# microsoft/typeagent-py

Measured on AMD Instinct MI355X. Metric: queries/sec + p50 lookup latency, 1536-d top-32 kNN at 1/2/4/8 MI355X, higher is better.
Workload: dtype f16 storage, f32 accumulate; 1 GPU; cfg3: 10000000x1536 fp16, 1024 q/step, top-32, min_score 0; total_rows=10000000, k=32, parallelism=single GPU

## Files before the change

include/tavb.h:

```cpp
#ifndef TAVB_H
#define TAVB_H

#include <stdint.h>

#ifdef __cplusplus
extern "C" {
#endif

#define TAVB_ABI_VERSION 7

#define TAVB_OK 0
#define TAVB_E_INVALID (-1)
#define TAVB_E_HIP (-2)
#define TAVB_E_NO_CORPUS (-3)
#define TAVB_E_UNSUPPORTED (-4)
#define TAVB_E_NOMEM (-5)
#define TAVB_E_TIMEOUT (-7)
#define TAVB_E_PEER (-6)

#define TAVB_F32 0
#define TAVB_F16 1

#define TAVB_MAX_FUSED_K 256
#define TAVB_MAX_LARGE_K 16384
// ... 98 lines not shown
#define TAVB_KERNEL_MFMA 2
#define TAVB_KERNEL_NORMALIZE 3
#define TAVB_KERNEL_CONVERT 4
#define TAVB_KERNEL_MFMA_SAMPLE 5
#define TAVB_KERNEL_SKINNY 6
#define TAVB_KERNEL_RESCORE 7
#define TAVB_KERNEL_EXCHANGE 8
#define TAVB_KERNEL_TOPK 9
#define TAVB_KERNEL_COUNT 10
int tavb_profile_enable(tavb_ctx* ctx, int32_t on);
int tavb_profile_reset(tavb_ctx* ctx);
int tavb_profile_read(tavb_ctx* ctx, int32_t kernel_id, double* out_total_ms, int64_t* out_launches);

int tavb_plan_ladder(int64_t rows, int32_t nq, int32_t n_cu, int64_t* out_bounds, int32_t cap);

#ifdef __cplusplus
}
#endif
#endif
```

typeagent_py_amd/_native.py:

```python

from __future__ import annotations

import ctypes
import os
import threading
from ctypes import POINTER, byref, c_char_p, c_double, c_float, c_int, c_int32, c_int64, c_uint64, c_void_p

import numpy as np

ABI_VERSION = 7
TAVB_F32 = 0
TAVB_F16 = 1
MAX_FUSED_K = 256
MAX_LARGE_K = 16384
MAX_STREAM_QUERIES = 8

KERNEL_SCAN, KERNEL_MERGE, KERNEL_MFMA, KERNEL_NORMALIZE, KERNEL_CONVERT, KERNEL_MFMA_SAMPLE, KERNEL_SKINNY, KERNEL_RESCORE, KERNEL_EXCHANGE, KERNEL_TOPK = range(10)
COMM_ID_BYTES = 128

_LIB_NAME = os.environ.get("TAVB_LIBRARY", "libtavb.so")
_lib = None
_lib_lock = threading.Lock()

_SIGNATURES = [
# ... 37 lines not shown
    ("tavb_search_device", c_int, [c_void_p, c_void_p, c_int32, c_int32, c_float, c_void_p]),
    ("tavb_search_subset_device", c_int, [c_void_p, c_void_p, c_void_p, c_int64, c_int32, c_float, c_void_p]),
    ("tavb_search_subset_resident", c_int, [c_void_p, c_void_p, c_void_p, c_int64, c_int32, c_float, c_void_p, c_void_p, c_void_p]),
    ("tavb_merge_device", c_int, [c_void_p, c_void_p, c_int32, c_int32, c_int32, c_void_p]),
    ("tavb_decode_keys", c_int, [c_void_p, c_int32, c_int32, c_void_p, c_void_p, c_void_p]),
    ("tavb_comm_unique_id", c_int, [c_void_p]),
    ("tavb_comm_init", c_int, [c_void_p, c_void_p, c_int32, c_int32]),
    ("tavb_comm_destroy", c_int, [c_void_p]),
    ("tavb_search_allgather", c_int, [c_void_p, c_void_p, c_int32, c_int32, c_float, c_void_p]),
    ("tavb_allgather_merge", c_int, [c_void_p, c_void_p, c_int32, c_int32, c_void_p]),
    ("tavb_remap_key_positions", c_int, [c_void_p, c_void_p, c_int64, c_void_p, c_int64]),
    ("tavb_profile_enable", c_int, [c_void_p, c_int32]),
    ("tavb_profile_reset", c_int, [c_void_p]),
    ("tavb_profile_read", c_int, [c_void_p, c_int32, POINTER(c_double), POINTER(c_int64)]),
    ("tavb_plan_ladder", c_int, [c_int64, c_int32, c_int32, POINTER(c_int64), c_int32]),
]

ABI_SYMBOLS = [name for name, _, _ in _SIGNATURES]


_AS_POINTER = ctypes.c_char * 0


def _addr(arr: np.ndarray):
    try:
        return _AS_POINTER.from_buffer(arr)
    except (TypeError, ValueError, BufferError):
        return arr.ctypes.data_as(c_void_p)


def plan_ladder(rows: int, nq: int, n_cu: int = 256) -> list[int]:
    lib = load_library(preload_torch=False)
    buf = (c_int64 * 16)()
    n = lib.tavb_plan_ladder(int(rows), int(nq), int(n_cu), buf, 16)
    _check(lib, n if n < 0 else 0)
    return [int(buf[i]) for i in range(n + 1)]


def library_path() -> str:
    return os.path.join(os.path.dirname(os.path.abspath(__file__)), _LIB_NAME)


def load_library(preload_torch: bool = True):
    global _lib
    with _lib_lock:
        if _lib is not None:
            return _lib
        path = library_path()
        if not os.path.isfile(path):
            raise RuntimeError(
                f"{path} is missing: build it with `python -c 'import __graft_entry__ as g; g.build()'` "
# ... 558 lines not shown
```

typeagent_py_amd/csrc/tavb_abi.hip:

```cpp

#include <hip/hip_runtime.h>
#include <dlfcn.h>
#include <rccl/rccl.h>

#include <algorithm>
#include <atomic>
#include <chrono>
#include <functional>
#include <mutex>
#include <cmath>
#include <cstdarg>
#include <cstdio>
#include <cstring>
#include <string>
#include <thread>
#include <vector>

#include "tavb_internal.h"

typedef unsigned long long u64_t;

namespace {

thread_local std::string g_last_error;
// ... 118 lines not shown
  Buffer d_sort_keys, d_sort_ws;
  Buffer h_sort_info{nullptr, 0, true};
  int64_t sort_all = 1;
  int64_t sort_stage_keys = (int64_t)1 << 21;
  int64_t sort_small_keys = 16384;
  Buffer h_ring[2] = {{nullptr, 0, true}, {nullptr, 0, true}};
  Buffer d_ring[2];
  hipEvent_t ring_done[2] = {nullptr, nullptr};
  const int32_t* row_to_msg = nullptr;
  int64_t row_to_msg_rows = 0, n_messages = 0;
  int64_t norm_rows = 0;
  Buffer h_stage{nullptr, 0, true};
  Buffer h_out{nullptr, 0, true};
  Buffer h_lists{nullptr, 0, true};
  Buffer h_flag{nullptr, 0, true};
  int64_t mfma_bdirect = 0;
  int64_t band_max = tavb::kBandMax;
  int64_t early_exact = 1;
  int64_t wide_fallback = 1;
  int64_t small_direct_bytes = (int64_t)128 << 20;
  int64_t small_direct_keys = 8192;
  int64_t last_direct = 0;
  int inline_query = 1;
  int64_t direct_group_max_nq = TAVB_MAX_GROUPED_QUERIES;
  int64_t direct_group = 0;
  int64_t direct_group_wgs = 0;
  bool dispatch_no_group = false;
  int64_t direct_group_keys = 32768;

  bool profiling = false;
// ... 435 lines not shown
  } else if (n == "mfma_ablate") {
    if (v < 0 || v > 4095) return fail(TAVB_E_INVALID, "mfma_ablate must be 0..4095");
    c->mfma_ablate = v;
  } else if (n == "mfma_splits") {
    if (v < 0 || v > 4096) return fail(TAVB_E_INVALID, "mfma_splits out of range");
    c->mfma_splits = v;
  } else if (n == "band_max") {
    if (v < TAVB_MAX_FUSED_K || v > tavb::kBandMax) return fail(TAVB_E_INVALID, "band_max must be %d .. %d", TAVB_MAX_FUSED_K, tavb::kBandMax);
    c->band_max = v;
  } else if (n == "early_exact") {
    c->early_exact = v ? 1 : 0;
  } else if (n == "wide_fallback") {
    c->wide_fallback = v ? 1 : 0;
  } else if (n == "mfma_bdirect") {
    c->mfma_bdirect = v ? 1 : 0;
  } else if (n == "small_direct_keys") {
    if (v < 64 || v > (1 << 20)) return fail(TAVB_E_INVALID, "small_direct_keys must be 64 .. 1048576");
    c->small_direct_keys = v;
  } else if (n == "inline_query") {
    c->inline_query = v ? 1 : 0;
  } else if (n == "direct_group_max_nq") {
    if (v < 0 || v > TAVB_MAX_GROUPED_QUERIES) return fail(TAVB_E_INVALID, "direct_group_max_nq must be 0 .. %d", TAVB_MAX_GROUPED_QUERIES);
    c->direct_group_max_nq = v;
  } else if (n == "direct_group") {
    if (!(v == 0 || v == 1 || v == 2 || v == 4 || v == 8)) return fail(TAVB_E_INVALID, "direct_group must be 0, 1, 2, 4 or 8");
    c->direct_group = v;
  } else if (n == "direct_group_wgs") {
    if (v != 0 && (v < 8 || v > 65536)) return fail(TAVB_E_INVALID, "direct_group_wgs must be 0 or 8 .. 65536");
    c->direct_group_wgs = v;
  } else if (n == "direct_group_keys") {
// ... 83 lines not shown
  else if (n == "small_direct_bytes") *out = c->small_direct_bytes;
  else if (n == "wide_fallback") *out = c->wide_fallback;
  else if (n == "early_exact") *out = c->early_exact;
  else if (n == "band_max") *out = c->band_max;
  else if (n == "last_doomed") {
    *out = 0;
    if (c->d_flag.ptr) {
      DeviceGuard guard(c->device);
      int v = 0;
      TAVB_HIP(hipStreamSynchronize(c->stream));
      TAVB_HIP(hipMemcpy(&v, reinterpret_cast<const int*>(c->d_flag.ptr) + 1, sizeof v, hipMemcpyDeviceToHost));
      *out = v;
    }
  }
  else if (n == "mfma_bdirect") *out = c->mfma_bdirect;
  else if (n == "last_direct") *out = c->last_direct;
  else if (n == "inline_query") *out = c->inline_query;
  else if (n == "small_direct_keys") *out = c->small_direct_keys;
  else if (n == "direct_group_max_nq") *out = c->direct_group_max_nq;
  else if (n == "direct_group") *out = c->direct_group;
  else if (n == "direct_group_wgs") *out = c->direct_group_wgs;
  else if (n == "direct_group_keys") *out = c->direct_group_keys;
  else if (n == "graph_max_bytes") *out = c->graph_max_bytes;
  else if (n == "last_graph") *out = c->last_graph;
  else if (n == "large_k") *out = c->large_k;
  else if (n == "topk_buckets") *out = c->topk_buckets;
  else if (n == "topk_boundary_keys") *out = c->topk_boundary_keys;
  else if (n == "topk_scores_bytes") *out = c->topk_scores_bytes;
  else if (n == "last_topk_refine") *out = c->last_topk_refine;
  else if (n == "sort_all") *out = c->sort_all;
// ... 1496 lines not shown
  p.nq_padded = r.nq_pad;
  p.k = k;
  p.index_base = r.index_base;
  p.min_score = r.kernel_min_score;
  p.n_splits = splits;
  p.ablate = (int)c->mfma_ablate;
  p.sched = (int)c->mfma_sched;
  p.f32 = r.q32 ? 1 : 0;
  p.skinny_tile = r.skinny ? r.qt : 0;
  p.wide_tile = r.skinny ? 0 : r.qt;
  p.active = r.active;
  p.active_min = r.active_min;
  p.active_max = r.active_max;
  p.split_plane = r.split_plane;
  p.bdirect = r.bdirect ? 1 : 0;
  const std::vector<int64_t> bounds = ladder_bounds(c->rows, splits, r.nq_pad, r.skinny, r.ladder, c->mfma_sample_rows, c->mfma_ladder);
  const int n_phases = (int)bounds.size() - 1;
  const int kc = wide ? (int)c->band_max : k;
  if (wide)
    if (int rc = c->d_thr.reserve((size_t)r.nq_pad * sizeof(float))) return rc;
  if (n_phases > 1 || (wide && r.active)) {
    if (int rc = c->d_thr.reserve((size_t)r.nq_pad * sizeof(float))) return rc;
    if (int rc = c->d_sample_keys.reserve((size_t)2 * nq * kc * sizeof(u64_t) + (size_t)2 * nq * sizeof(int))) return rc;
  }
  p.band = r.band;
  p.lost = r.lost;
  const float* floor = r.floor;
  const size_t row_bytes = (size_t)dim * (r.q32 ? 4 : 2);
  for (int ph = 0; ph < n_phases; ++ph) {
    const bool last = (ph == n_phases - 1);
// ... 15 lines not shown
    }
    u64_t* const running = reinterpret_cast<u64_t*>(c->d_sample_keys.ptr);
    const u64_t* const run_in = running ? running + (size_t)((ph + 1) & 1) * nq * kc : nullptr;
    u64_t* const run_out = running ? running + (size_t)(ph & 1) * nq * kc : nullptr;
    int* const run_cnt = running ? reinterpret_cast<int*>(running + (size_t)2 * nq * kc) : nullptr;
    const int* const cnt_in = run_cnt ? run_cnt + (size_t)((ph + 1) & 1) * nq : nullptr;
    int* const cnt_out = run_cnt ? run_cnt + (size_t)(ph & 1) * nq : nullptr;
    if (carried && !wide) {
      TAVB_HIP(hipMemcpy2DAsync(pp.lists + (size_t)pp.n_splits * k, (size_t)pp.list_stride * k * sizeof(u64_t), run_in,
                                (size_t)k * sizeof(u64_t), (size_t)k * sizeof(u64_t), (size_t)nq, hipMemcpyDeviceToDevice, c->stream));
    }
    {
      Timed t(c, r.active ? TAVB_KERNEL_RESCORE : !last ? TAVB_KERNEL_MFMA_SAMPLE : (r.skinny ? TAVB_KERNEL_SKINNY : TAVB_KERNEL_MFMA));
      hipError_t e = launch(pp);
      if (e != hipSuccess) return fail(TAVB_E_HIP, "mfma scan launch failed (phase %d): %s", ph, hipGetErrorString(e));
    }
    if (wide) {
      Timed t(c, r.active ? TAVB_KERNEL_RESCORE : TAVB_KERNEL_MERGE);
      float* d_thr = reinterpret_cast<float*>(c->d_thr.ptr);
      u64_t* const last_out = r.active ? run_out : d_out;
      int* const last_cnt = r.active ? cnt_out : r.band_cnt;
      hipError_t e = tavb::launch_select_band(pp.workspace, pp.counts, pp.n_splits, nq, r.nq_pad, k, kc, carried ? run_in : nullptr, carried ? cnt_in : nullptr,
                                              floor, r.band, last ? last_out : run_out, last ? last_cnt : cnt_out, (last && r.active) ? nullptr : d_thr, r.lost,
                                              last ? r.verdict : nullptr, c->stream, r.active, r.active_min, r.active_max > 0 ? r.active_max : 0x7fffffff,
                                              doom_gate ? r.doomed : nullptr, r.doomed_max, doom_count ? r.doomed : nullptr, doom_limit);
      if (e != hipSuccess) return fail(TAVB_E_HIP, "select launch failed: %s", hipGetErrorString(e));
      if (last && r.active) {
        e = tavb::launch_rescore_slots(c->corpus, false, c->dim, r.index_base, r.rs_queries, last_out, kc, last_cnt, r.rs_min_scores, nq, k, d_out,
                                       scatter, r.active, r.active_min, r.active_max > 0 ? r.active_max : 0x7fffffff, c->stream);
        if (e != hipSuccess) return fail(TAVB_E_HIP, "fallback rescore launch failed: %s", hipGetErrorString(e));
// ... 332 lines not shown
    r.q32 = q32;
    r.qt = qt;
    r.nq = nq;
    r.nq_pad = nq_pad;
    r.k = k;
    r.index_base = index_base;
    r.kernel_min_score = uniform_thr ? min_scores[0] : lowest_min_score(min_scores, nq);
    r.floor = d_ms_floor;
    r.queries = c->d_queries_f16.ptr;
    r.ladder = true;
    return run_tile_ladder(c, r, d_out, nullptr);
  }
  return search_device_impl(c, d_q, nq, k, min_scores, nullptr, c->rows, index_base, d_out);
}

extern "C" int tavb_plan_ladder(int64_t rows, int32_t nq, int32_t n_cu, int64_t* out_bounds, int32_t cap) {
  if (rows < 0 || nq < 1 || n_cu < 8) return fail(TAVB_E_INVALID, "bad shape");
  const int qt = tavb::mfma_query_tile_for(nq, rows, n_cu);
  const int nq_pad = ((nq + qt - 1) / qt) * qt;
  const int splits = tavb::mfma_pick_splits(rows, nq_pad, qt, n_cu);
  const std::vector<int64_t> b = ladder_bounds(rows, splits, nq_pad, false, true, 0, 4);
  for (size_t i = 0; out_bounds && i < b.size() && (int)i < cap; ++i) out_bounds[i] = b[i];
  return (int)b.size() - 1;
}
```

typeagent_py_amd/csrc/tavb_internal.h:

```cpp
#pragma once

#include <hip/hip_runtime.h>
#include <stddef.h>
#include <stdint.h>

#include "../../include/tavb.h"

#define TAVB_MAX_GROUPED_QUERIES 128

namespace tavb {

struct ScanParams {
  const void* corpus;
  const int32_t* row_ids;
  const float* queries;
  unsigned long long* lists;
  int64_t n_pos;
  int32_t dim;
  int32_t dtype;
  int32_t nq;
  int32_t k;
  uint32_t index_base;
  unsigned long long key_bound;
  int32_t group;
// ... 117 lines not shown
  int32_t sched;
  int32_t ablate;
  const float* thr_in;
  const int* active;
  int32_t active_min;
  int32_t active_max;
  const int* gate;
  int32_t gate_max;
  int32_t bdirect;
  int64_t split_plane;
  int32_t f32;
  int32_t skinny_tile;
  int32_t wide_tile;
  const float* band;
  unsigned* lost;
};
hipError_t launch_mfma_scan(const MfmaParams& p, hipStream_t stream);
hipError_t launch_sample_thresholds(const unsigned long long* keys, int nq, int k, const float* floor, float* thr, hipStream_t stream);
int mfma_query_tile(int nq);
int mfma_query_tile_for(int nq, int64_t rows, int n_cu);
int mfma_pick_splits(int64_t rows, int nq_padded, int tile, int n_cu);
bool mfma_supported(int dim, int k);
size_t mfma_workspace_bytes(int n_splits, int nq_padded, bool wide);
constexpr int kBandMax = 2048;
hipError_t launch_select_band(const unsigned long long* cand, const int* counts, int n_splits, int nq, int nq_padded, int k, int kc_max,
                              const unsigned long long* carried, const int* carried_cnt, const float* floor, const float* band, unsigned long long* out,
                              int* out_cnt, float* thr_out, unsigned* lost, int* verdict, hipStream_t stream, const int* active = nullptr,
                              int active_min = 0, int active_max = 0x7fffffff, const int* gate = nullptr, int gate_max = 0, int* doomed = nullptr,
                              int doom_limit = 0);
hipError_t launch_skinny_scan(const MfmaParams& p, hipStream_t stream);
int skinny_query_tile(int nq);
int skinny_pick_splits(int64_t rows, int nq_padded, int tile, int n_cu, int dim, bool f32, int sched);
// ... 4 lines not shown
```

typeagent_py_amd/csrc/tavb_mfma.hip:

```cpp

#include <hip/hip_runtime.h>

#include <type_traits>

#include "tavb_device.h"
#include "tavb_internal.h"

namespace tavb {

namespace {

constexpr int BM = 256;
constexpr int BN = 256;
constexpr int BK = 64;
constexpr int CAP = 512;
constexpr int CAPW = 1024;

typedef float f32x16 __attribute__((ext_vector_type(16)));
typedef __attribute__((address_space(3))) void lds_void;
typedef const __attribute__((address_space(1))) void global_void;

struct MfmaDeviceParams {
  const _Float16* corpus;
  const _Float16* queries;
// ... 231 lines not shown
  static constexpr int CTRL = B_RING + 2 * SLOT_B;
  static constexpr int LDS = CTRL + QT * 8 + 16;
  static constexpr int PIECES_B = QT / 8 / 4;
  static constexpr int PIECES = PIECES_A6 + PIECES_B;
};

template <int NT, int N3, int N0, int N1>
constexpr int staging_piece_at(int q, int i) {
  const int n = q == 3 ? N3 : q == 0 ? N0 : q == 1 ? N1 : 0;
  const int base = q == 3 ? 0 : q == 0 ? N3 : N3 + N0;
  for (int j = 0; j < n; ++j)
    if ((j * NT + NT / 2) / n == i) return base + j;
  return -1;
}

template <int ABL, int NI, int N3, int N0, int N1, bool SPLIT = false, bool BD = false>
__global__ void __launch_bounds__(NT6) mfma_scan_kernel(const MfmaDeviceParams p) {
  using G = WideGeom<NI>;
  constexpr int BN = G::QT, NT = G::NT, SLOT_B6 = G::SLOT_B, PIECES_B6 = G::PIECES_B, B_RING6 = G::B_RING;
  constexpr int RA = BD ? 3 : G::RA;
  constexpr int CTRL6 = BD ? 3 * SLOT_A6 : G::CTRL;
  constexpr int PIECES6 = BD ? PIECES_A6 : G::PIECES;
  static_assert(!BD || (NI == 4 && !SPLIT), "the direct query operand is built for the 256-query tile");
  static_assert(N3 + N0 + N1 == PIECES6, "every piece of a step is issued exactly once");
  static_assert(N3 <= NT && N0 <= NT && N1 <= NT && NI + 5 <= NT, "one piece / one fragment read behind an MFMA at most");
  extern __shared__ __align__(16) unsigned char smem[];
  float* thr_lds = reinterpret_cast<float*>(smem + CTRL6);
  int* cnt_lds = reinterpret_cast<int*>(smem + CTRL6 + BN * 4);
  typedef __attribute__((address_space(3))) volatile int lds_flag;
  lds_flag* need_compact = (lds_flag*)(smem + CTRL6 + BN * 8);

  const int tid = threadIdx.x;
  const int wave = __builtin_amdgcn_readfirstlane(tid >> 6);
  const int wm = wave >> 1;
  const int wn = wave & 1;

  const int b = blockIdx.x;
  const int xcd = b & 7;
  const int t = b >> 3;
  const int qtile = t % p.n_qtiles;
// ... 25 lines not shown

  const int D = p.dim;
  const int steps_per_plane = D / 64;
  const int steps_per_tile = SPLIT ? 2 * steps_per_plane : steps_per_plane;
  const uint32_t row_bytes = (uint32_t)D * 2u;
  const char* corpus = reinterpret_cast<const char*>(p.corpus);
  const char* qbase = reinterpret_cast<const char*>(p.queries) + (size_t)qtile * BN * row_bytes;
  const int n_tiles = (r_end > r_begin) ? (int)((r_end - r_begin + BM6 - 1) / BM6) : 0;
  if (n_tiles == 0) {
    for (int i = tid; i < BN; i += NT6) my_counts[i] = 0;
    return;
  }

  int st_even, st_odd;
  uint32_t frag_x, a_lane, b_lane;
  {
    int zero = 0;
    asm volatile("" : "+v"(zero));
    const int ln = (int)__builtin_amdgcn_mbcnt_hi(~0u, __builtin_amdgcn_mbcnt_lo(~0u, (unsigned)zero));
    const uint32_t lane_row = (uint32_t)(ln >> 3);
    st_even = (int)(lane_row * row_bytes + (uint32_t)(((ln & 7) ^ (ln >> 4)) * 16));
    st_odd = (int)(lane_row * row_bytes + (uint32_t)(((ln & 7) ^ (4 + (ln >> 4))) * 16));
    const int frag_row = ln & 31;
    frag_x = (uint32_t)(((ln >> 5) ^ ((frag_row >> 1) & 7)) << 4);
    a_lane = (uint32_t)((wm * 160 + frag_row) * 128);
    b_lane = (uint32_t)(B_RING6 + (wn * G::WQ + frag_row) * 128);
  }
  const __amdgpu_buffer_rsrc_t rsrc_b =
      __builtin_amdgcn_make_buffer_rsrc(const_cast<char*>(sgpr_ptr(qbase)), 0, (int)(BN * row_bytes) + (SPLIT ? (int)p.split_plane : 0), 0x00020000);
  const int plane_jump = SPLIT ? (int)p.split_plane - steps_per_plane * 128 : 0;

  int sa_kt = 0, sa_tile = 0, sa_slot = 0;
  int sb_kt = 0, sb_slot = 0;
  auto stage_a = [&](auto j_tag) {
    constexpr int J = decltype(j_tag)::value;
    const int tile = sa_tile < n_tiles ? sa_tile : n_tiles - 1;
    const int64_t row0 = (ABL & 4) ? 0 : r_begin + (int64_t)tile * BM6;
    const int64_t left = p.rows - row0;
    const int valid = (int)(left < BM6 ? left : BM6);
    const __amdgpu_buffer_rsrc_t rsrc_a = __builtin_amdgcn_make_buffer_rsrc(
        const_cast<char*>(sgpr_ptr(corpus + (size_t)row0 * row_bytes)), 0, __builtin_amdgcn_readfirstlane(valid * (int)row_bytes), 0x00020000);
// ... 37 lines not shown
  auto stage_a_all = [&]<int... I>(std::integer_sequence<int, I...>) { (stage_a(std::integral_constant<int, I>{}), ...); };

  if constexpr (RA == 2) {
    stage_range(std::make_integer_sequence<int, PIECES6>{});
    stage_range(std::make_integer_sequence<int, N3>{});
    wait_vmcnt<N3>();
  } else {
    stage_a_all(std::make_integer_sequence<int, PIECES_A6>{});
    stage_range(std::make_integer_sequence<int, PIECES6>{});
    stage_range(std::make_integer_sequence<int, N3>{});
    wait_vmcnt<PIECES_A6 + N3>();
  }
  __syncthreads();

  typedef int i32x4 __attribute__((ext_vector_type(4)));
  constexpr int NA_TILES = G::NA;
  f32x16 acc_a[NA_TILES];
  f32x16 acc_v[NT - NA_TILES > 0 ? NT - NA_TILES : 1];
#define TAVB_MFMA6_A(ACC, A, B) \
  asm volatile("v_mfma_f32_32x32x16_f16 %0, %1, %2, %0" : "+a"(ACC) : "v"(__builtin_bit_cast(i32x4, A)), "v"(__builtin_bit_cast(i32x4, B)))
#define TAVB_MFMA6_V(ACC, A, B) \
  asm volatile("v_mfma_f32_32x32x16_f16 %0, %1, %2, %0" : "+v"(ACC) : "v"(__builtin_bit_cast(i32x4, A)), "v"(__builtin_bit_cast(i32x4, B)))
#define TAVB_MFMA6_A0(ACC, A, B) \
  asm volatile("v_mfma_f32_32x32x16_f16 %0, %1, %2, 0" : "=a"(ACC) : "v"(__builtin_bit_cast(i32x4, A)), "v"(__builtin_bit_cast(i32x4, B)))
#define TAVB_MFMA6_V0(ACC, A, B) \
  asm volatile("v_mfma_f32_32x32x16_f16 %0, %1, %2, 0" : "=&v"(ACC) : "v"(__builtin_bit_cast(i32x4, A)), "v"(__builtin_bit_cast(i32x4, B)))

  f16x8 a0[5], b0[NI], a1[5], b1[NI];
  f16x8 b2[BD ? NI : 1], b3[BD ? NI : 1];
  constexpr int BQ_SLICE = (BN / 32) * 1024;
  int bq_soff = 0;
  const int bq_tile_bytes = BN * (int)row_bytes;
  int bq_voff = 0;
  auto bq_load = [&](f16x8(&dst)[BD ? NI : 1]) {
    if constexpr (BD) {
#pragma unroll
      for (int ni = 0; ni < NI; ++ni)
        dst[ni] = __builtin_bit_cast(f16x8, __builtin_amdgcn_raw_buffer_load_b128(rsrc_b, bq_voff + ni * 1024, bq_soff, 0));
      bq_soff = (bq_soff + BQ_SLICE == bq_tile_bytes) ? 0 : bq_soff + BQ_SLICE;
    }
  };
  {
    const unsigned char* abase = smem + (a_lane + frag_x);
    const unsigned char* bbase = smem + (b_lane + frag_x);
    if constexpr (BD) {
      int zero_b = 0;
      asm volatile("" : "+v"(zero_b));
      const int ln_b = (int)__builtin_amdgcn_mbcnt_hi(~0u, __builtin_amdgcn_mbcnt_lo(~0u, (unsigned)zero_b));
      bq_voff = ln_b * 16 + wn * NI * 1024;
      bq_load(b0);
      bq_load(b1);
      bq_load(b2);
    } else {
#pragma unroll
      for (int ni = 0; ni < NI; ++ni) b0[ni] = *reinterpret_cast<const f16x8*>(bbase + ni * 4096);
    }
#pragma unroll
    for (int mi = 0; mi < 5; ++mi) a0[mi] = *reinterpret_cast<const f16x8*>(abase + mi * 4096);
  }
  int rd = 0, rd_a = 0;

  auto quarter = [&](auto q_tag, auto first_tag, f16x8(&fa)[5], f16x8(&fb)[NI], f16x8(&na)[5], f16x8(&nb)[NI], int nslot_a, int nslot, auto nkk_tag) {
    constexpr int Q = decltype(q_tag)::value;
    constexpr bool FIRST = decltype(first_tag)::value;
    constexpr int NKK = decltype(nkk_tag)::value;
    const uint32_t kx = (uint32_t)(NKK << 5) ^ frag_x;
    const unsigned char* abase = smem + nslot_a * SLOT_A6 + (a_lane + kx);
    const unsigned char* bbase = smem + nslot * SLOT_B6 + (b_lane + kx);
    auto mfma_at = [&](auto i_tag) {
      constexpr int I = decltype(i_tag)::value;
      constexpr bool BMAJ = (ABL & 1024) != 0, SERP = (ABL & 2048) != 0;
      constexpr int outer = BMAJ ? I / 5 : I / NI;
      constexpr int inner0 = BMAJ ? I % 5 : I % NI;
// ... 19 lines not shown
        } else {
          if constexpr (I < NI) nb[I] = *reinterpret_cast<const f16x8*>(bbase + I * 4096);
        }
        if constexpr (I >= NI && I < NI + 5) na[I - NI] = *reinterpret_cast<const f16x8*>(abase + (I - NI) * 4096);
      }
      if constexpr ((ABL & 2) == 0) {
        constexpr int PC = staging_piece_at<NT, N3, N0, N1>(Q, I);
        if constexpr (PC >= 0) stage_piece(std::integral_constant<int, PC>{});
      }
    };
    [&]<int... I>(std::integer_sequence<int, I...>) { (mfma_at(std::integral_constant<int, I>{}), ...); }
    (std::make_integer_sequence<int, NT>{});
    if constexpr (BD) bq_soff = (bq_soff + BQ_SLICE == bq_tile_bytes) ? 0 : bq_soff + BQ_SLICE;
    if constexpr ((ABL & 1) != 0) asm volatile("" ::"v"(fa[0]), "v"(fa[4]), "v"(fb[0]), "v"(fb[NI - 1]));
  };
  using Q0 = std::integral_constant<int, 0>;
  using Q1 = std::integral_constant<int, 1>;
  using Q2 = std::integral_constant<int, 2>;
  using Q3 = std::integral_constant<int, 3>;
  auto step = [&](auto first_tag) {
    if constexpr (BD) {
      quarter(Q0{}, first_tag, a0, b0, a1, b3, rd_a, rd, Q1{});
      quarter(Q1{}, std::false_type{}, a1, b1, a0, b0, rd_a, rd, Q2{});
      quarter(Q2{}, std::false_type{}, a0, b2, a1, b1, rd_a, rd, Q3{});
      if constexpr ((ABL & 2) == 0) wait_vmcnt<5 * NI + PIECES_A6>();
      __builtin_amdgcn_s_waitcnt(0xC07F);
      TAVB_BARRIER();
      const int nxt_a = rd_a + 1 == RA ? 0 : rd_a + 1;
      quarter(Q3{}, std::false_type{}, a1, b3, a0, b2, nxt_a, rd, Q0{});
      rd_a = nxt_a;
    } else {
      quarter(Q0{}, first_tag, a0, b0, a1, b1, rd_a, rd, Q1{});
      quarter(Q1{}, std::false_type{}, a1, b1, a0, b0, rd_a, rd, Q2{});
      quarter(Q2{}, std::false_type{}, a0, b0, a1, b1, rd_a, rd, Q3{});
      if constexpr ((ABL & 2) == 0) wait_vmcnt<(RA == 2 ? 0 : PIECES_A6)>();
      __builtin_amdgcn_s_waitcnt(0xC07F);
      TAVB_BARRIER();
      const int nxt_a = (RA == 2) ? (rd_a ^ 1) : (rd_a + 1 == RA ? 0 : rd_a + 1);
      quarter(Q3{}, std::false_type{}, a1, b1, a0, b0, nxt_a, rd ^ 1, Q0{});
      rd ^= 1;
      rd_a = nxt_a;
    }
  };

  for (int tile = 0; tile < n_tiles; ++tile) {
    const int64_t row0 = r_begin + (int64_t)tile * BM6;
    const bool tile_full = row0 + BM6 <= r_end;
    if constexpr ((ABL & 1) != 0) {
#pragma unroll
      for (int i = 0; i < NA_TILES; ++i)
#pragma unroll
        for (int r = 0; r < 16; ++r) acc_a[i][r] = 0.f;
#pragma unroll
      for (int i = 0; i < NT - NA_TILES; ++i)
#pragma unroll
        for (int r = 0; r < 16; ++r) acc_v[i][r] = 0.f;
    }
    step(std::true_type{});
#pragma unroll 1
    for (int kt = 1; kt < steps_per_tile; ++kt) step(std::false_type{});

    asm volatile("s_nop 15\n\ts_nop 15" ::: "memory");
    int zero_e = 0;
    asm volatile("" : "+v"(zero_e));
    const int lane_e = (int)__builtin_amdgcn_mbcnt_hi(~0u, __builtin_amdgcn_mbcnt_lo(~0u, (unsigned)zero_e));
#pragma unroll
    for (int pass = 0; pass < 2; ++pass)
#pragma unroll
      for (int ni = 0; ni < NI; ++ni) {
        const int ql = wn * G::WQ + ni * 32 + (lane_e & 31);
        const float thr = thr_lds[ql];
        const float thr_pre = fmaf(thr, 2.0f, -1.0f) - 4.8e-7f;
#pragma unroll
        for (int mi = 0; mi < 5; ++mi) {
          constexpr int VT = NT - NA_TILES > 0 ? NT - NA_TILES : 1;
          if ((mi * NI + ni >= NA_TILES) != (pass == 0)) continue;
          const f32x16 dots = (mi * NI + ni < NA_TILES) ? acc_a[mi * NI + ni] : acc_v[(mi * NI + ni - NA_TILES + VT) % VT];
          float top = dots[0];
#pragma unroll
          for (int r = 1; r < 16; ++r) top = __builtin_fmaxf(top, dots[r]);
// ... 19 lines not shown
              for (int j = 0; j < 4; ++j) {
                const int r_off = j + 8 * g;
                if (m[j] == 0ull) continue;
                if (((m[j] >> lane_e) & 1ull) != 0ull && r_off < rows_left) {
                  const int pos = lds_add_rtn(&cnt_lds[ql], 1);
                  if (pos + 1 > CAPW - BM6) lds_store_i32(need_compact, 1);
                  float s1 = (sc[j] > 0.0f) ? sc[j] : 0.0f;
                  s1 = (s1 > 1.0f) ? 1.0f : s1;
                  if (pos < CAPW) my_cand[(size_t)ql * CAPW + pos] = make_key(s1, (uint32_t)(row_base + r_off) + p.index_base);
                }
              }
            }
          }
        }
      }
    asm volatile("s_waitcnt lgkmcnt(0)" ::: "memory");
    TAVB_BARRIER();
    if (*need_compact != 0) {
      asm volatile("s_waitcnt vmcnt(0)" ::: "memory");
      TAVB_BARRIER();
      for (int q = wave; q < BN; q += NT6 / 64) {
        const int n = cnt_lds[q];
        if (n > CAPW - BM6) {
          u64* buf = my_cand + (size_t)q * CAPW;
          const int qg = qtile * BN + q;
          const float band = p.band ? p.band[qg] : 0.0f;
          float thr_excl;
          uint32_t lost;
          const int kept = compact_to_band<CAPW>(buf, n < CAPW ? n : CAPW, p.k, lane_e, band, CAPW - BM6 - 64, &thr_excl, &lost);
          if (lane_e == 0) {
// ... 656 lines not shown
size_t mfma_workspace_bytes(int n_splits, int nq_padded, bool wide) {
  return (size_t)n_splits * (size_t)nq_padded * (wide ? CAPW : CAP) * sizeof(u64);
}

hipError_t launch_select_band(const unsigned long long* cand, const int* counts, int n_splits, int nq, int nq_padded, int k, int kc_max,
                              const unsigned long long* carried, const int* carried_cnt, const float* floor, const float* band, unsigned long long* out,
                              int* out_cnt, float* thr_out, unsigned* lost, int* verdict, hipStream_t stream, const int* active, int active_min,
                              int active_max, const int* gate, int gate_max, int* doomed, int doom_limit) {
  if (nq < 1 || k < 1 || k > TAVB_MAX_FUSED_K || n_splits < 1 || n_splits > 256 || nq_padded < nq || kc_max < k || kc_max > SEL_CACHE / 2 || kc_max > kBandMax) return hipErrorInvalidValue;
  constexpr int lds = SEL_CACHE * (int)sizeof(u64);
  hipError_t e = ensure_dynamic_lds(reinterpret_cast<const void*>(select_band_kernel), lds);
  if (e != hipSuccess) return e;
  hipLaunchKernelGGL(select_band_kernel, dim3(nq), dim3(256), lds, stream, cand, counts, n_splits, nq_padded, k, kc_max, carried, carried_cnt, floor, band,
                     out, out_cnt, thr_out, lost, verdict, active, active_min, active_max, gate, gate_max, doomed, doom_limit);
  return hipGetLastError();
}

hipError_t launch_mfma_scan(const MfmaParams& p, hipStream_t stream) {
  const int tile = p.wide_tile == 128 ? 128 : BN;
  if (!mfma_supported(p.dim, p.k) || p.nq_padded % tile != 0 || p.n_splits < 1) return hipErrorInvalidValue;
  MfmaDeviceParams d{};
  d.corpus = reinterpret_cast<const _Float16*>(p.corpus);
  d.queries = reinterpret_cast<const _Float16*>(p.queries);
  d.lists = p.lists;
  d.rows = p.rows;
  d.dim = p.dim;
  d.nq = p.nq;
  d.n_qtiles = p.nq_padded / tile;
  d.n_splits = p.n_splits;
  d.list_stride = p.list_stride > p.n_splits ? p.list_stride : p.n_splits;
// ... 27 lines not shown
    if (p.dim % 64 != 0) return hipErrorInvalidValue;
    constexpr int LDS256 = WideGeom<4>::LDS, LDS128 = WideGeom<2>::LDS;
    if (p.split_plane > 0) {
      if (tile != BN) return hipErrorInvalidValue;
      return go(mfma_scan_kernel<0, 4, 8, 6, 4, true>, NT6, LDS256);
    }
    if (tile == 128) {
      switch (p.ablate) {
        case 1: return go(mfma_scan_kernel<1, 2, 6, 4, 4>, NT6, LDS128);
        case 256: return go(mfma_scan_kernel<256, 2, 6, 4, 4>, NT6, LDS128);
        case 257: return go(mfma_scan_kernel<257, 2, 6, 4, 4>, NT6, LDS128);
        case 264: return go(mfma_scan_kernel<264, 2, 6, 4, 4>, NT6, LDS128);
        default: return go(mfma_scan_kernel<0, 2, 6, 4, 4>, NT6, LDS128);
      }
    }
    if (p.bdirect && p.ablate == 0) return go(mfma_scan_kernel<0, 4, 4, 3, 3, false, true>, NT6, 3 * SLOT_A6 + BN * 8 + 16);
    switch (p.ablate) {
      case 256: return go(mfma_scan_kernel<256, 4, 8, 6, 4>, NT6, LDS256);
      case 260: return go(mfma_scan_kernel<260, 4, 8, 6, 4>, NT6, LDS256);
      case 264: return go(mfma_scan_kernel<264, 4, 8, 6, 4>, NT6, LDS256);
      case 268: return go(mfma_scan_kernel<268, 4, 8, 6, 4>, NT6, LDS256);
      case 258: return go(mfma_scan_kernel<258, 4, 8, 6, 4>, NT6, LDS256);
      case 1282: return go(mfma_scan_kernel<1282, 4, 8, 6, 4>, NT6, LDS256);
      case 2306: return go(mfma_scan_kernel<2306, 4, 8, 6, 4>, NT6, LDS256);
      case 3330: return go(mfma_scan_kernel<3330, 4, 8, 6, 4>, NT6, LDS256);
      default: break;
    }
    switch (p.sched) {
      case 1: return go(mfma_scan_kernel<0, 4, 10, 8, 0>, NT6, LDS256);
      case 2: return go(mfma_scan_kernel<0, 4, 6, 6, 6>, NT6, LDS256);
// ... 106 lines not shown
```

Before: 40900 queries/s.

## Add 16x16x32 MFMA variant of the 256-query wide scan kernel

Adds an M16 template path to the wide MFMA scan kernel that uses v_mfma_f32_16x16x32_f16 with 80 four-register accumulators instead of 32x32x16 tiles. It brings new fragment addressing, a restructured quarter schedule of 40 MFMAs per quarter with reload-distance static asserts, and a matching threshold/candidate epilogue. The new mfma_shape option defaults to 16, so the default 256-tile, non-split path now launches this kernel. The smaller MFMA shape may change issue density, register pressure and LDS read traffic, and the epilogue does more, smaller ballot checks.

```diff
diff --git a/include/tavb.h b/include/tavb.h
--- a/include/tavb.h
+++ b/include/tavb.h
@@ -136,6 +136,8 @@
 
 int tavb_plan_ladder(int64_t rows, int32_t nq, int32_t n_cu, int64_t* out_bounds, int32_t cap);
 
+int tavb_plan_filter_shape(int32_t shape, int32_t query_tile, int32_t split, int32_t bdirect, int32_t sched, int32_t ablate);
+
 #ifdef __cplusplus
 }
 #endif
diff --git a/typeagent_py_amd/_native.py b/typeagent_py_amd/_native.py
--- a/typeagent_py_amd/_native.py
+++ b/typeagent_py_amd/_native.py
@@ -75,6 +75,7 @@
     ("tavb_profile_reset", c_int, [c_void_p]),
     ("tavb_profile_read", c_int, [c_void_p, c_int32, POINTER(c_double), POINTER(c_int64)]),
     ("tavb_plan_ladder", c_int, [c_int64, c_int32, c_int32, POINTER(c_int64), c_int32]),
+    ("tavb_plan_filter_shape", c_int, [c_int32, c_int32, c_int32, c_int32, c_int32, c_int32]),
 ]
 
 ABI_SYMBOLS = [name for name, _, _ in _SIGNATURES]
@@ -96,6 +97,13 @@
     n = lib.tavb_plan_ladder(int(rows), int(nq), int(n_cu), buf, 16)
     _check(lib, n if n < 0 else 0)
     return [int(buf[i]) for i in range(n + 1)]
+
+
+def plan_filter_shape(shape: int, query_tile: int = 256, split: bool = False, bdirect: bool = False, sched: int = 0, ablate: int = 0) -> int:
+    lib = load_library(preload_torch=False)
+    r = lib.tavb_plan_filter_shape(int(shape), int(query_tile), int(bool(split)), int(bool(bdirect)), int(sched), int(ablate))
+    _check(lib, r if r < 0 else 0)
+    return int(r)
 
 
 def library_path() -> str:
diff --git a/typeagent_py_amd/csrc/tavb_abi.hip b/typeagent_py_amd/csrc/tavb_abi.hip
--- a/typeagent_py_amd/csrc/tavb_abi.hip
+++ b/typeagent_py_amd/csrc/tavb_abi.hip
@@ -156,6 +156,8 @@
   Buffer h_out{nullptr, 0, true};
   Buffer h_lists{nullptr, 0, true};
   Buffer h_flag{nullptr, 0, true};
+  int64_t mfma_shape = 16;
+  int64_t last_mfma_shape = 0;
   int64_t mfma_bdirect = 0;
   int64_t band_max = tavb::kBandMax;
   int64_t early_exact = 1;
@@ -621,6 +623,9 @@
     c->wide_fallback = v ? 1 : 0;
   } else if (n == "mfma_bdirect") {
     c->mfma_bdirect = v ? 1 : 0;
+  } else if (n == "mfma_shape") {
+    if (tavb_plan_filter_shape((int32_t)v, 256, 0, 0, 0, 0) < 0) return TAVB_E_INVALID;
+    c->mfma_shape = v;
   } else if (n == "small_direct_keys") {
     if (v < 64 || v > (1 << 20)) return fail(TAVB_E_INVALID, "small_direct_keys must be 64 .. 1048576");
     c->small_direct_keys = v;
@@ -734,6 +739,8 @@
     }
   }
   else if (n == "mfma_bdirect") *out = c->mfma_bdirect;
+  else if (n == "mfma_shape") *out = c->mfma_shape;
+  else if (n == "last_mfma_shape") *out = c->last_mfma_shape;
   else if (n == "last_direct") *out = c->last_direct;
   else if (n == "inline_query") *out = c->inline_query;
   else if (n == "small_direct_keys") *out = c->small_direct_keys;
@@ -2260,6 +2267,7 @@
   p.active_max = r.active_max;
   p.split_plane = r.split_plane;
   p.bdirect = r.bdirect ? 1 : 0;
+  p.shape = (int)c->mfma_shape;
   const std::vector<int64_t> bounds = ladder_bounds(c->rows, splits, r.nq_pad, r.skinny, r.ladder, c->mfma_sample_rows, c->mfma_ladder);
   const int n_phases = (int)bounds.size() - 1;
   const int kc = wide ? (int)c->band_max : k;
@@ -2305,6 +2313,7 @@
       Timed t(c, r.active ? TAVB_KERNEL_RESCORE : !last ? TAVB_KERNEL_MFMA_SAMPLE : (r.skinny ? TAVB_KERNEL_SKINNY : TAVB_KERNEL_MFMA));
       hipError_t e = launch(pp);
       if (e != hipSuccess) return fail(TAVB_E_HIP, "mfma scan launch failed (phase %d): %s", ph, hipGetErrorString(e));
+      if (wide && pp.split_plane == 0) c->last_mfma_shape = tavb::mfma_tile_shape(pp);
     }
     if (wide) {
       Timed t(c, r.active ? TAVB_KERNEL_RESCORE : TAVB_KERNEL_MERGE);
@@ -2667,6 +2676,19 @@
   return search_device_impl(c, d_q, nq, k, min_scores, nullptr, c->rows, index_base, d_out);
 }
 
+extern "C" int tavb_plan_filter_shape(int32_t shape, int32_t query_tile, int32_t split, int32_t bdirect, int32_t sched, int32_t ablate) {
+  if (shape != 16 && shape != 32) return fail(TAVB_E_INVALID, "mfma_shape must be 16 or 32");
+  if (query_tile != 128 && query_tile != 256) return fail(TAVB_E_INVALID, "query_tile must be 128 or 256");
+  tavb::MfmaParams p{};
+  p.shape = shape;
+  p.wide_tile = query_tile;
+  p.split_plane = split ? 1 : 0;
+  p.bdirect = bdirect ? 1 : 0;
+  p.sched = sched;
+  p.ablate = ablate;
+  return tavb::mfma_tile_shape(p);
+}
+
 extern "C" int tavb_plan_ladder(int64_t rows, int32_t nq, int32_t n_cu, int64_t* out_bounds, int32_t cap) {
   if (rows < 0 || nq < 1 || n_cu < 8) return fail(TAVB_E_INVALID, "bad shape");
   const int qt = tavb::mfma_query_tile_for(nq, rows, n_cu);
diff --git a/typeagent_py_amd/csrc/tavb_internal.h b/typeagent_py_amd/csrc/tavb_internal.h
--- a/typeagent_py_amd/csrc/tavb_internal.h
+++ b/typeagent_py_amd/csrc/tavb_internal.h
@@ -155,8 +155,10 @@
   int32_t wide_tile;
   const float* band;
   unsigned* lost;
+  int32_t shape;
 };
 hipError_t launch_mfma_scan(const MfmaParams& p, hipStream_t stream);
+int mfma_tile_shape(const MfmaParams& p);
 hipError_t launch_sample_thresholds(const unsigned long long* keys, int nq, int k, const float* floor, float* thr, hipStream_t stream);
 int mfma_query_tile(int nq);
 int mfma_query_tile_for(int nq, int64_t rows, int n_cu);
diff --git a/typeagent_py_amd/csrc/tavb_mfma.hip b/typeagent_py_amd/csrc/tavb_mfma.hip
--- a/typeagent_py_amd/csrc/tavb_mfma.hip
+++ b/typeagent_py_amd/csrc/tavb_mfma.hip
@@ -269,7 +269,16 @@
   return -1;
 }
 
-template <int ABL, int NI, int N3, int N0, int N1, bool SPLIT = false, bool BD = false>
+constexpr int m16_query_frag(int i) { return i / 5; }
+constexpr int m16_row_frag(int i) { return i % 5; }
+constexpr int m16_last_reader(bool query, int f) {
+  int last = -1;
+  for (int i = 0; i < 40; ++i)
+    if ((query ? m16_query_frag(i) : m16_row_frag(i)) == f) last = i;
+  return last;
+}
+
+template <int ABL, int NI, int N3, int N0, int N1, bool SPLIT = false, bool BD = false, bool M16 = false>
 __global__ void __launch_bounds__(NT6) mfma_scan_kernel(const MfmaDeviceParams p) {
   using G = WideGeom<NI>;
   constexpr int BN = G::QT, NT = G::NT, SLOT_B6 = G::SLOT_B, PIECES_B6 = G::PIECES_B, B_RING6 = G::B_RING;
@@ -277,8 +286,10 @@
   constexpr int CTRL6 = BD ? 3 * SLOT_A6 : G::CTRL;
   constexpr int PIECES6 = BD ? PIECES_A6 : G::PIECES;
   static_assert(!BD || (NI == 4 && !SPLIT), "the direct query operand is built for the 256-query tile");
+  static_assert(!M16 || (NI == 4 && !SPLIT && !BD), "the 16x16x32 form is built for the 256-query filter tile");
+  constexpr int QM = M16 ? 40 : NT;
   static_assert(N3 + N0 + N1 == PIECES6, "every piece of a step is issued exactly once");
-  static_assert(N3 <= NT && N0 <= NT && N1 <= NT && NI + 5 <= NT, "one piece / one fragment read behind an MFMA at most");
+  static_assert(N3 <= QM && N0 <= QM && N1 <= QM && NI + 5 <= NT, "one piece / one fragment read behind an MFMA at most");
   extern __shared__ __align__(16) unsigned char smem[];
   float* thr_lds = reinterpret_cast<float*>(smem + CTRL6);
   int* cnt_lds = reinterpret_cast<int*>(smem + CTRL6 + BN * 4);
@@ -334,6 +345,7 @@
 
   int st_even, st_odd;
   uint32_t frag_x, a_lane, b_lane;
+  uint32_t frag_x16, a_lane16, b_lane16;
   {
     int zero = 0;
     asm volatile("" : "+v"(zero));
@@ -345,6 +357,10 @@
     frag_x = (uint32_t)(((ln >> 5) ^ ((frag_row >> 1) & 7)) << 4);
     a_lane = (uint32_t)((wm * 160 + frag_row) * 128);
     b_lane = (uint32_t)(B_RING6 + (wn * G::WQ + frag_row) * 128);
+    const int frag_row16 = ln & 15;
+    frag_x16 = (uint32_t)(((ln >> 4) ^ ((frag_row16 >> 1) & 7)) << 4);
+    a_lane16 = (uint32_t)((wm * 160 + frag_row16) * 128);
+    b_lane16 = (uint32_t)(B_RING6 + (wn * G::WQ + frag_row16) * 128);
   }
   const __amdgpu_buffer_rsrc_t rsrc_b =
       __builtin_amdgcn_make_buffer_rsrc(const_cast<char*>(sgpr_ptr(qbase)), 0, (int)(BN * row_bytes) + (SPLIT ? (int)p.split_plane : 0), 0x00020000);
@@ -412,9 +428,11 @@
   __syncthreads();
 
   typedef int i32x4 __attribute__((ext_vector_type(4)));
-  constexpr int NA_TILES = G::NA;
-  f32x16 acc_a[NA_TILES];
-  f32x16 acc_v[NT - NA_TILES > 0 ? NT - NA_TILES : 1];
+  using Acc = std::conditional_t<M16, f32x4, f32x16>;
+  constexpr int NACC = M16 ? 80 : NT;
+  constexpr int NA_TILES = M16 ? 60 : G::NA;
+  Acc acc_a[NA_TILES];
+  Acc acc_v[NACC - NA_TILES > 0 ? NACC - NA_TILES : 1];
 #define TAVB_MFMA6_A(ACC, A, B) \
   asm volatile("v_mfma_f32_32x32x16_f16 %0, %1, %2, %0" : "+a"(ACC) : "v"(__builtin_bit_cast(i32x4, A)), "v"(__builtin_bit_cast(i32x4, B)))
 #define TAVB_MFMA6_V(ACC, A, B) \
@@ -423,8 +441,16 @@
   asm volatile("v_mfma_f32_32x32x16_f16 %0, %1, %2, 0" : "=a"(ACC) : "v"(__builtin_bit_cast(i32x4, A)), "v"(__builtin_bit_cast(i32x4, B)))
 #define TAVB_MFMA6_V0(ACC, A, B) \
   asm volatile("v_mfma_f32_32x32x16_f16 %0, %1, %2, 0" : "=&v"(ACC) : "v"(__builtin_bit_cast(i32x4, A)), "v"(__builtin_bit_cast(i32x4, B)))
-
-  f16x8 a0[5], b0[NI], a1[5], b1[NI];
+#define TAVB_MFMA16_A(ACC, A, B) \
+  asm volatile("v_mfma_f32_16x16x32_f16 %0, %1, %2, %0" : "+a"(ACC) : "v"(__builtin_bit_cast(i32x4, A)), "v"(__builtin_bit_cast(i32x4, B)))
+#define TAVB_MFMA16_V(ACC, A, B) \
+  asm volatile("v_mfma_f32_16x16x32_f16 %0, %1, %2, %0" : "+v"(ACC) : "v"(__builtin_bit_cast(i32x4, A)), "v"(__builtin_bit_cast(i32x4, B)))
+#define TAVB_MFMA16_A0(ACC, A, B) \
+  asm volatile("v_mfma_f32_16x16x32_f16 %0, %1, %2, 0" : "=a"(ACC) : "v"(__builtin_bit_cast(i32x4, A)), "v"(__builtin_bit_cast(i32x4, B)))
+#define TAVB_MFMA16_V0(ACC, A, B) \
+  asm volatile("v_mfma_f32_16x16x32_f16 %0, %1, %2, 0" : "=&v"(ACC) : "v"(__builtin_bit_cast(i32x4, A)), "v"(__builtin_bit_cast(i32x4, B)))
+
+  f16x8 a0[5], b0[M16 ? 2 * NI : NI], a1[5], b1[M16 ? 1 : NI];
   f16x8 b2[BD ? NI : 1], b3[BD ? NI : 1];
   constexpr int BQ_SLICE = (BN / 32) * 1024;
   int bq_soff = 0;
@@ -449,12 +475,21 @@
       bq_load(b0);
       bq_load(b1);
       bq_load(b2);
+    } else if constexpr (M16) {
+      const unsigned char* abase16 = smem + (a_lane16 + frag_x16);
+      const unsigned char* bbase16 = smem + (b_lane16 + frag_x16);
+#pragma unroll
+      for (int n = 0; n < 2 * NI; ++n) b0[n] = *reinterpret_cast<const f16x8*>(bbase16 + n * 2048);
+#pragma unroll
+      for (int m = 0; m < 5; ++m) a0[m] = *reinterpret_cast<const f16x8*>(abase16 + m * 2048);
     } else {
 #pragma unroll
       for (int ni = 0; ni < NI; ++ni) b0[ni] = *reinterpret_cast<const f16x8*>(bbase + ni * 4096);
     }
-#pragma unroll
-    for (int mi = 0; mi < 5; ++mi) a0[mi] = *reinterpret_cast<const f16x8*>(abase + mi * 4096);
+    if constexpr (!M16) {
+#pragma unroll
+      for (int mi = 0; mi < 5; ++mi) a0[mi] = *reinterpret_cast<const f16x8*>(abase + mi * 4096);
+    }
   }
   int rd = 0, rd_a = 0;
 
@@ -504,12 +539,72 @@
     if constexpr (BD) bq_soff = (bq_soff + BQ_SLICE == bq_tile_bytes) ? 0 : bq_soff + BQ_SLICE;
     if constexpr ((ABL & 1) != 0) asm volatile("" ::"v"(fa[0]), "v"(fa[4]), "v"(fb[0]), "v"(fb[NI - 1]));
   };
+  auto quarter16 = [&](auto q_tag, auto first_tag, f16x8(&fa)[5], f16x8(&na)[5], int nslot_a, int nslot, auto nkk_tag) {
+    constexpr int Q = decltype(q_tag)::value;
+    constexpr bool FIRST = decltype(first_tag)::value;
+    constexpr int NKK = decltype(nkk_tag)::value;
+    constexpr int H = Q & 1;
+    const uint32_t kx = (uint32_t)(NKK << 6) ^ frag_x16;
+    const unsigned char* abase = smem + nslot_a * SLOT_A6 + (a_lane16 + (H ^ 1) * 5 * 2048 + kx);
+    const unsigned char* bbase = smem + nslot * SLOT_B6 + (b_lane16 + kx);
+    auto mfma_at = [&](auto i_tag) {
+      constexpr int I = decltype(i_tag)::value;
+      constexpr int n = m16_query_frag(I), m = m16_row_frag(I), mr = 5 * H + m;
+      constexpr bool VB = mr >= 5 && n >= 4;
+      constexpr int J = VB ? (mr - 5) * 4 + (n - 4) : (mr < 5 ? mr * 8 + n : 40 + (mr - 5) * 4 + n);
+      if constexpr ((ABL & 1) == 0) {
+        if constexpr (FIRST) {
+          if constexpr (VB)
+            TAVB_MFMA16_V0(acc_v[J], fa[m], b0[n]);
+          else
+            TAVB_MFMA16_A0(acc_a[J], fa[m], b0[n]);
+        } else {
+          if constexpr (VB)
+            TAVB_MFMA16_V(acc_v[J], fa[m], b0[n]);
+          else
+            TAVB_MFMA16_A(acc_a[J], fa[m], b0[n]);
+        }
+      }
+      if constexpr ((ABL & 32) == 0) {
+        if constexpr (I < 5) {
+          static_assert(I + QM - m16_last_reader(false, I) >= 5, "five MFMAs between the last read of a row fragment and its reload");
+          na[I] = *reinterpret_cast<const f16x8*>(abase + I * 2048);
+        }
+        if constexpr ((Q & 1) == 1 && I >= 9 && (I - 9) % 5 == 0) {
+          static_assert(I - m16_last_reader(true, (I - 9) / 5) >= 5, "five MFMAs between the last read of a query fragment and its reload");
+          b0[(I - 9) / 5] = *reinterpret_cast<const f16x8*>(bbase + ((I - 9) / 5) * 2048);
+        }
+        if constexpr ((Q & 1) == 0 && I == 5) {
+          static_assert(I + QM - m16_last_reader(true, 7) >= 5, "five MFMAs between the last read of a query fragment and its reload");
+          b0[7] = *reinterpret_cast<const f16x8*>(bbase + 7 * 2048);
+        }
+      }
+      if constexpr ((ABL & 2) == 0) {
+        constexpr int PC = staging_piece_at<QM, N3, N0, N1>(Q, I);
+        if constexpr (PC >= 0) stage_piece(std::integral_constant<int, PC>{});
+      }
+    };
+    [&]<int... I>(std::integer_sequence<int, I...>) { (mfma_at(std::integral_constant<int, I>{}), ...); }
+    (std::make_integer_sequence<int, QM>{});
+    if constexpr ((ABL & 1) != 0) asm volatile("" ::"v"(fa[0]), "v"(fa[4]), "v"(b0[0]), "v"(b0[7]));
+  };
   using Q0 = std::integral_constant<int, 0>;
   using Q1 = std::integral_constant<int, 1>;
   using Q2 = std::integral_constant<int, 2>;
   using Q3 = std::integral_constant<int, 3>;
   auto step = [&](auto first_tag) {
-    if constexpr (BD) {
+    if constexpr (M16) {
+      quarter16(Q0{}, first_tag, a0, a1, rd_a, rd, Q0{});
+      quarter16(Q1{}, first_tag, a1, a0, rd_a, rd, Q1{});
+      quarter16(Q2{}, std::false_type{}, a0, a1, rd_a, rd, Q1{});
+      if constexpr ((ABL & 2) == 0) wait_vmcnt<0>();
+      __builtin_amdgcn_s_waitcnt(0xC07F);
+      TAVB_BARRIER();
+      const int nxt_a = rd_a ^ 1;
+      quarter16(Q3{}, std::false_type{}, a1, a0, nxt_a, rd ^ 1, Q0{});
+      rd ^= 1;
+      rd_a = nxt_a;
+    } else if constexpr (BD) {
       quarter(Q0{}, first_tag, a0, b0, a1, b3, rd_a, rd, Q1{});
       quarter(Q1{}, std::false_type{}, a1, b1, a0, b0, rd_a, rd, Q2{});
       quarter(Q2{}, std::false_type{}, a0, b2, a1, b1, rd_a, rd, Q3{});
@@ -538,13 +633,9 @@
     const bool tile_full = row0 + BM6 <= r_end;
     if constexpr ((ABL & 1) != 0) {
 #pragma unroll
-      for (int i = 0; i < NA_TILES; ++i)
-#pragma unroll
-        for (int r = 0; r < 16; ++r) acc_a[i][r] = 0.f;
-#pragma unroll
-      for (int i = 0; i < NT - NA_TILES; ++i)
-#pragma unroll
-        for (int r = 0; r < 16; ++r) acc_v[i][r] = 0.f;
+      for (int i = 0; i < NA_TILES; ++i) acc_a[i] = Acc{};
+#pragma unroll
+      for (int i = 0; i < NACC - NA_TILES; ++i) acc_v[i] = Acc{};
     }
     step(std::true_type{});
 #pragma unroll 1
@@ -554,6 +645,65 @@
     int zero_e = 0;
     asm volatile("" : "+v"(zero_e));
     const int lane_e = (int)__builtin_amdgcn_mbcnt_hi(~0u, __builtin_amdgcn_mbcnt_lo(~0u, (unsigned)zero_e));
+    if constexpr (M16) {
+#pragma unroll
+      for (int pass = 0; pass < 2; ++pass)
+#pragma unroll
+        for (int n = 0; n < 8; ++n) {
+          const int ql = wn * G::WQ + n * 16 + (lane_e & 15);
+          const float thr = thr_lds[ql];
+          const float thr_pre = fmaf(thr, 2.0f, -1.0f) - 4.8e-7f;
+#pragma unroll
+          for (int h = 0; h < 2; ++h) {
+            constexpr int VT = NACC - NA_TILES;
+            const bool vb = h == 1 && n >= 4;
+            if (vb != (pass == 0)) continue;
+            f32x4 dots[5];
+#pragma unroll
+            for (int m = 0; m < 5; ++m) {
+              const int mr = 5 * h + m;
+              dots[m] = vb ? acc_v[((mr - 5) * 4 + (n - 4) + VT) % VT] : acc_a[(mr < 5 ? mr * 8 + n : 40 + (mr - 5) * 4 + n) % NA_TILES];
+            }
+            float top = dots[0][0];
+#pragma unroll
+            for (int m = 0; m < 5; ++m)
+#pragma unroll
+              for (int r = 0; r < 4; ++r) top = __builtin_fmaxf(top, dots[m][r]);
+            TAVB_SB();
+            const bool any = ((ABL & ~3072) == 0 || ABL == 512) && (top > thr_pre);
+            if constexpr (ABL == 512) asm volatile("" ::"s"(__builtin_amdgcn_ballot_w64(any)));
+            if constexpr ((ABL & ~3072) != 0 && ABL != 512) asm volatile("" ::"v"(top));
+            if (ABL != 512 && __builtin_amdgcn_ballot_w64(any) != 0ull) {
+              const int64_t row_base = row0 + wm * 160 + h * 80 + 4 * (lane_e >> 4);
+              const int64_t left64 = r_end - row_base;
+              const int rows_left = tile_full ? 80 : (int)(left64 < 80 ? left64 : 80);
+#pragma unroll
+              for (int m = 0; m < 5; ++m) {
+                float sc[4];
+                u64 mk[4];
+#pragma unroll
+                for (int j = 0; j < 4; ++j) {
+                  sc[j] = fmaf(dots[m][j], 0.5f, 0.5f);
+                  asm volatile("v_cmp_gt_f32 %0, %1, %2" : "=s"(mk[j]) : "v"(sc[j]), "v"(thr));
+                }
+                if ((mk[0] | mk[1] | mk[2] | mk[3]) == 0ull) continue;
+#pragma unroll
+                for (int j = 0; j < 4; ++j) {
+                  const int r_off = 16 * m + j;
+                  if (mk[j] == 0ull) continue;
+                  if (((mk[j] >> lane_e) & 1ull) != 0ull && r_off < rows_left) {
+                    const int pos = lds_add_rtn(&cnt_lds[ql], 1);
+                    if (pos + 1 > CAPW - BM6) lds_store_i32(need_compact, 1);
+                    float s1 = (sc[j] > 0.0f) ? sc[j] : 0.0f;
+                    s1 = (s1 > 1.0f) ? 1.0f : s1;
+                    if (pos < CAPW) my_cand[(size_t)ql * CAPW + pos] = make_key(s1, (uint32_t)(row_base + r_off) + p.index_base);
+                  }
+                }
+              }
+            }
+          }
+        }
+    } else {
 #pragma unroll
     for (int pass = 0; pass < 2; ++pass)
 #pragma unroll
@@ -603,6 +753,7 @@
           }
         }
       }
+    }
     asm volatile("s_waitcnt lgkmcnt(0)" ::: "memory");
     TAVB_BARRIER();
     if (*need_compact != 0) {
@@ -1289,6 +1440,12 @@
   hipLaunchKernelGGL(select_band_kernel, dim3(nq), dim3(256), lds, stream, cand, counts, n_splits, nq_padded, k, kc_max, carried, carried_cnt, floor, band,
                      out, out_cnt, thr_out, lost, verdict, active, active_min, active_max, gate, gate_max, doomed, doom_limit);
   return hipGetLastError();
+}
+
+int mfma_tile_shape(const MfmaParams& p) {
+  if (p.shape != 16 || p.wide_tile == 128 || p.split_plane > 0) return 32;
+  if (p.ablate != 0) return (p.ablate == 256 || p.ablate == 258) ? 16 : 32;
+  return (p.bdirect || p.sched != 0) ? 32 : 16;
 }
 
 hipError_t launch_mfma_scan(const MfmaParams& p, hipStream_t stream) {
@@ -1346,6 +1503,13 @@
         default: return go(mfma_scan_kernel<0, 2, 6, 4, 4>, NT6, LDS128);
       }
     }
+    if (mfma_tile_shape(p) == 16) {
+      switch (p.ablate) {
+        case 256: return go(mfma_scan_kernel<256, 4, 8, 6, 4, false, false, true>, NT6, LDS256);
+        case 258: return go(mfma_scan_kernel<258, 4, 8, 6, 4, false, false, true>, NT6, LDS256);
+        default: return go(mfma_scan_kernel<0, 4, 8, 6, 4, false, false, true>, NT6, LDS256);
+      }
+    }
     if (p.bdirect && p.ablate == 0) return go(mfma_scan_kernel<0, 4, 4, 3, 3, false, true>, NT6, 3 * SLOT_A6 + BN * 8 + 16);
     switch (p.ablate) {
       case 256: return go(mfma_scan_kernel<256, 4, 8, 6, 4>, NT6, LDS256);
```

Result: faster. 42310 queries/s (median of 6 runs) (+3.4%).
